# gabry1998/Self-Supervised-Anomaly-Detection

Hardware: AMD Instinct MI355X
Metric: train images/sec + anomaly-maps/sec, ResNet-18 256x256 bs256 (higher is better)
Workload: dtype f32; 1 GPU; ResNet-18 256x256 bs256 self-sup train + anomaly map, 1xMI355X, synthetic images (BASELINE configs[1]); images_per_gpu=256, global_batch=256, patches_per_image=841, bank_rows=588, parallelism=dp1 (256 images), train_step_launch=hipGraph segments, train_graph_segments=1

## Files before the change

### include/ssad.h

```cpp
#ifndef SSAD_H
#define SSAD_H
#include <stddef.h>
#include <stdint.h>

#ifdef __cplusplus
extern "C" {
#endif

#define SSAD_VERSION 100

int ssad_version(void);
const char* ssad_last_error(void);

int ssad_repack_oihw_to_ohwi(const float* w_oihw, float* w_ohwi, int O, int I, int KH, int KW, void* stream);
int ssad_repack_ohwi_to_oihw(const float* w_ohwi, float* w_oihw, int O, int I, int KH, int KW, void* stream);
int ssad_pack_stem_weight(const float* w_oihw, float* wk, void* stream);
int ssad_pack_stem_weight_ohwi(const float* w_ohwi, float* wk, void* stream);

int ssad_stem_fwd(const float* img, int B, int H, int W, int patch_dim, int patch_stride, int Hv, int Wv,
                  const float* wk, const float* scale, const float* shift, int relu, int hwnc, float* out, void* stream);
int ssad_stem_stats_rows(void);
int ssad_stem_fwd_stats(const float* img, int B, int H, int W, int Hv, int Wv, const float* wk, float* out, float eps,
                        float momentum, float* mean, float* invstd, float* running_mean, float* running_var, double* workspace,
                        void* stream);

int ssad_pack_stem_weight_folded(const float* w_oihw, float* wf, void* stream);
int ssad_stem_patch_pool_fwd(const float* img, int B, int H, int W, int patch_stride, const float* wf, const float* scale,
                             const float* shift, int hwnc, float* out, void* stream);
int ssad_stem_patch_pool_fwd_ring(const float* img, int B, int H, int W, int patch_stride, const float* wf, const float* scale,
                                  const float* shift, int hwnc, int skip_lo, int skip_hi, float* out, void* stream);
int ssad_stem_patch_border_fwd(const float* img, int B, int H, int W, int patch_stride, const float* wf, const float* scale,
                               const float* shift, float* out, void* stream);

int ssad_maxpool3x3s2_fwd(const float* in, float* out, int64_t N, int H, int W, int C, int hwnc, void* stream);

int ssad_conv_igemm_fwd(const float* in, const float* w_ohwi, float* out, const float* scale, const float* shift,
                        const float* residual, int relu, int64_t N, int H, int W, int Cin, int Cout, int KH, int KW,
                        int stride, int pad, void* stream);

int ssad_conv_igemm_fwd_hwnc(const float* in, const float* w_ohwi, float* out, const float* scale, const float* shift,
                             const float* residual, int relu, int64_t N, int H, int W, int Cin, int Cout, int KH, int KW,
                             int stride, int pad, void* stream);

int ssad_conv_igemm_fwd_hwnc_ring(const float* in, const float* w_ohwi, float* out, const float* scale, const float* shift,
                                  const float* residual, int relu, int64_t N, int H, int W, int Cin, int Cout, int KH, int KW,
                                  int stride, int pad, int skip_lo, int skip_hi, void* stream);
int ssad_patch_gather_hwnc(const float* dense, float* out, int64_t B, int prow, int pcol, int shift, int Hd, int Wd, int C,
                           int H, int W, int lo, int hi, void* stream);
int ssad_patch_gather_hwnc_band(const float* dense, float* out, int64_t B, int prow, int pcol, int shift, int Hd, int Wd, int C,
                                int H, int W, int lo, int hi, int ilo, int ihi, void* stream);

int ssad_conv_igemm_tile(int64_t N, int H, int W, int Cin, int Cout, int KH, int KW, int stride, int pad, int mode);
int ssad_conv_igemm_tile_id(int64_t N, int H, int W, int Cin, int Cout, int KH, int KW, int stride, int pad, int mode);

int ssad_gap_fwd(const float* in, float* out, int64_t N, int HW, int C, int out_stride, int out_offset, int hwnc,
// ... 376 lines not shown
```

### self-supervised-anomaly-detection_amd/csrc/stem.hip

```cpp
#include "common.h"
#include <type_traits>

namespace {

constexpr int STEM_MAX_GRID = 4096;


constexpr int TOH = 8, TOW = 32;
constexpr int TIH = TOH * 2 + 5;
constexpr int TIW = 72;
constexpr int KSTEPS = 7 * 4 * 3;
constexpr int IN_TILE = TIH * TIW * 3;
constexpr int W_TILE = KSTEPS * 2 * 64;

struct StemParams {
    const float* img;
    const float* wk;
    const float* scale;
    const float* shift;
    float* out;
    int B, H, W, pd, ps, Hv, Wv, Ho, Wo, relu;
    int prow, pcol;
    int ph, pw;
    int tiles_y, tiles_x;
// ... 168 lines not shown
            const int which = tid >> 6, cc = tid & 63;
            p.stats[((int64_t)blockIdx.x * 2 + which) * 64 + cc] =
                ((S[(0 * 2 + which) * 64 + cc] + S[(1 * 2 + which) * 64 + cc]) + S[(2 * 2 + which) * 64 + cc]) + S[(3 * 2 + which) * 64 + cc];
        }
    }
}

constexpr int SP_SW = 40, SP_SH = 36;
constexpr int SP_SRC = SP_SH * SP_SW * 3;
constexpr int SP_WF = 24 * 2 * 64;
constexpr int SP_CB = 9 * 32 * 32;

struct StemPatchParams {
    const float* img;
    const float* wf;
    const float* scale;
    const float* shift;
    float* out;
    int B, H, W, ps, prow, pcol, hwnc;
    int skip_lo, skip_hi;
    int64_t Nsamp;
};

__global__ __launch_bounds__(256, 2) void stem_patch_fused_kernel(StemPatchParams p) {
    extern __shared__ __attribute__((aligned(16))) float lds[];
    float* wl = lds;
    float* src = lds + SP_WF;
    float* cb = src + SP_SRC;
    const int tid = threadIdx.x, lane = tid & 63, wave = tid >> 6;
    const int r = lane & 31, h = lane >> 5;
    for (int i = tid; i < SP_WF / 4; i += 256) ((f32x4*)wl)[i] = ((const f32x4*)p.wf)[i];
    const int P = p.prow * p.pcol;
    const int64_t plane = (int64_t)p.H * p.W;

    constexpr int NSRC = (SP_SH * SP_SW + 255) / 256;
    float pv[NSRC][3];
    auto fetch_patch = [&](int64_t n) {
        const int b = (int)(n / P);
        const int pi = (int)(n - (int64_t)b * P);
        const int y0 = (pi / p.pcol) * p.ps, x0 = (pi % p.pcol) * p.ps;
        const float* im = p.img + (int64_t)b * 3 * plane;
#pragma unroll
        for (int q = 0; q < NSRC; ++q) {
            const int i = tid + 256 * q;
            const int ty = i / SP_SW, tx = i - ty * SP_SW;
            const int sy = ty - 2, sx = tx - 2;
            float v0 = 0.f, v1 = 0.f, v2 = 0.f;
            if (i < SP_SH * SP_SW && (unsigned)sy < 32u && (unsigned)sx < 32u) {
                const float* s = im + (int64_t)(y0 + sy) * p.W + x0 + sx;
                v0 = s[0]; v1 = s[plane]; v2 = s[2 * plane];
            }
            pv[q][0] = v0; pv[q][1] = v1; pv[q][2] = v2;
        }
    };
    if ((int64_t)blockIdx.x < p.Nsamp) fetch_patch(blockIdx.x);
    for (int64_t n = blockIdx.x; n < p.Nsamp; n += gridDim.x) {
        __syncthreads();
#pragma unroll
        for (int q = 0; q < NSRC; ++q) {
            const int i = tid + 256 * q;
            if (i < SP_SH * SP_SW) {
                float* d = src + i * 3;
                d[0] = pv[q][0]; d[1] = pv[q][1]; d[2] = pv[q][2];
            }
        }
        if (n + gridDim.x < p.Nsamp) fetch_patch(n + gridDim.x);
        for (int pass = 0; pass < 2; ++pass) {
            const float sc = p.scale ? p.scale[pass * 32 + r] : 1.f;
            const float sh = p.shift ? p.shift[pass * 32 + r] : 0.f;
            for (int i = tid; i < 32 * 32; i += 256) cb[i] = 0.f;
            __syncthreads();
            for (int t = 0; t < 4; ++t) {
                f32x16 acc0, acc1;
#pragma unroll
                for (int e = 0; e < 16; ++e) { acc0[e] = 0.f; acc1[e] = 0.f; }
                const int oy = 8 * t + 2 * wave;
                const float* a0 = src + ((oy + 0) * SP_SW + r + h) * 3;
                const float* a1 = src + ((oy + 1) * SP_SW + r + h) * 3;
                const float* bw = wl + h * 64 + pass * 32 + r;
#pragma unroll
                for (int a = 0; a < 4; ++a)
#pragma unroll
                    for (int q = 0; q < 2; ++q)
#pragma unroll
                        for (int c = 0; c < 3; ++c) {
                            const int ko = (a * SP_SW + 2 * q) * 3 + c;
                            const float w = bw[((a * 2 + q) * 3 + c) * 128];
                            acc0 = mfma32(a0[ko], w, acc0);
                            acc1 = mfma32(a1[ko], w, acc1);
                        }
                float* c0 = cb + ((1 + 2 * wave) * 32) * 32 + r;
#pragma unroll
                for (int e = 0; e < 16; ++e) {
                    const int ox = (e & 3) + 8 * (e >> 2) + 4 * h;
                    c0[ox * 32] = fmaxf(acc0[e] * sc + sh, 0.f);
                    c0[(32 + ox) * 32] = fmaxf(acc1[e] * sc + sh, 0.f);
                }
                __syncthreads();
#pragma unroll
                for (int k = 0; k < 2; ++k) {
                    const int item = tid + 256 * k;
                    const int c4 = item & 7, px = (item >> 3) & 15, j = item >> 7;
                    if (4 * t + j >= p.skip_lo && 4 * t + j <= p.skip_hi && px >= p.skip_lo && px <= p.skip_hi) continue;
                    f32x4 m = {0.f, 0.f, 0.f, 0.f};
#pragma unroll
                    for (int dy = 0; dy < 3; ++dy)
#pragma unroll
                        for (int dx = -1; dx < 2; ++dx) {
                            const int cx = 2 * px + dx;
                            if (cx < 0) continue;
                            const f32x4 v = *(const f32x4*)(cb + ((2 * j + dy) * 32 + cx) * 32 + c4 * 4);
                            m[0] = fmaxf(m[0], v[0]); m[1] = fmaxf(m[1], v[1]); m[2] = fmaxf(m[2], v[2]); m[3] = fmaxf(m[3], v[3]);
                        }
                    const int py = 4 * t + j;
                    const int64_t pix = p.hwnc ? ((int64_t)py * 16 + px) * p.Nsamp + n : (n * 16 + py) * 16 + px;
                    *(f32x4*)(p.out + pix * 64 + pass * 32 + c4 * 4) = m;
                }
                __syncthreads();
                ((f32x4*)cb)[tid] = ((const f32x4*)(cb + 8 * 32 * 32))[tid];
                __syncthreads();
            }
        }
    }
}

constexpr int SB_CB = 7 * 32 * 32;

__global__ __launch_bounds__(256, 2) void stem_patch_border_kernel(StemPatchParams p) {
    extern __shared__ __attribute__((aligned(16))) float lds[];
    float* wl = lds;
    float* src = lds + SP_WF;
    float* cb = src + SP_SRC;
    const int tid = threadIdx.x, lane = tid & 63, wave = tid >> 6;
    const int r = lane & 31, h = lane >> 5;
    for (int i = tid; i < SP_WF / 4; i += 256) ((f32x4*)wl)[i] = ((const f32x4*)p.wf)[i];
    const int P = p.prow * p.pcol;
    const int64_t plane = (int64_t)p.H * p.W;
    constexpr int NSRC = (SP_SH * SP_SW + 255) / 256;
    float pv[NSRC][3];
    auto fetch_patch = [&](int64_t n) {
        const int b = (int)(n / P);
        const int pi = (int)(n - (int64_t)b * P);
        const int y0 = (pi / p.pcol) * p.ps, x0 = (pi % p.pcol) * p.ps;
        const float* im = p.img + (int64_t)b * 3 * plane;
#pragma unroll
        for (int q = 0; q < NSRC; ++q) {
            const int i = tid + 256 * q;
            const int ty = i / SP_SW, tx = i - ty * SP_SW;
            const int sy = ty - 2, sx = tx - 2;
            float v0 = 0.f, v1 = 0.f, v2 = 0.f;
            if (i < SP_SH * SP_SW && (unsigned)sy < 32u && (unsigned)sx < 32u) {
                const float* s = im + (int64_t)(y0 + sy) * p.W + x0 + sx;
                v0 = s[0]; v1 = s[plane]; v2 = s[2 * plane];
            }
            pv[q][0] = v0; pv[q][1] = v1; pv[q][2] = v2;
        }
    };
    auto row_of = [](int t) { return t < 4 ? t : 25 + t; };
    const int ta0 = 2 * wave, ta1 = 2 * wave + 1 < 7 ? 2 * wave + 1 : 2 * wave;
    const float* pa0 = src + (row_of(ta0) * SP_SW + r + h) * 3;
    const float* pa1 = src + (row_of(ta1) * SP_SW + r + h) * 3;
    const float *pb0, *pb1;
    {
        int q0 = (2 * wave) * 32 + r, q1 = (2 * wave + 1) * 32 + r;
        q0 = q0 < 189 ? q0 : 188; q1 = q1 < 189 ? q1 : 188;
        const int c0 = q0 % 7, c1 = q1 % 7;
        pb0 = src + ((3 + q0 / 7) * SP_SW + (c0 < 4 ? c0 : 25 + c0) + h) * 3;
        pb1 = src + ((3 + q1 / 7) * SP_SW + (c1 < 4 ? c1 : 25 + c1) + h) * 3;
    }
    auto two_tiles = [&](const float* a0, const float* a1, int pass, f32x16& acc0, f32x16& acc1) {
#pragma unroll
        for (int e = 0; e < 16; ++e) { acc0[e] = 0.f; acc1[e] = 0.f; }
        const float* bw = wl + h * 64 + pass * 32 + r;
#pragma unroll
        for (int a = 0; a < 4; ++a)
#pragma unroll
            for (int q = 0; q < 2; ++q)
#pragma unroll
                for (int c = 0; c < 3; ++c) {
                    const int ko = (a * SP_SW + 2 * q) * 3 + c;
                    const float w = bw[((a * 2 + q) * 3 + c) * 128];
                    acc0 = mfma32(a0[ko], w, acc0);
                    acc1 = mfma32(a1[ko], w, acc1);
                }
    };
    if ((int64_t)blockIdx.x < p.Nsamp) fetch_patch(blockIdx.x);
    for (int64_t n = blockIdx.x; n < p.Nsamp; n += gridDim.x) {
        __syncthreads();
#pragma unroll
        for (int q = 0; q < NSRC; ++q) {
            const int i = tid + 256 * q;
            if (i < SP_SH * SP_SW) {
                float* d = src + i * 3;
                d[0] = pv[q][0]; d[1] = pv[q][1]; d[2] = pv[q][2];
            }
        }
        if (n + gridDim.x < p.Nsamp) fetch_patch(n + gridDim.x);
        __syncthreads();
        for (int pass = 0; pass < 2; ++pass) {
            const float sc = p.scale ? p.scale[pass * 32 + r] : 1.f;
            const float sh = p.shift ? p.shift[pass * 32 + r] : 0.f;
            f32x16 acc0, acc1;
            two_tiles(pa0, pa1, pass, acc0, acc1);
#pragma unroll
            for (int e = 0; e < 16; ++e) {
                const int ox = (e & 3) + 8 * (e >> 2) + 4 * h;
                cb[((2 * wave) * 32 + ox) * 32 + r] = fmaxf(acc0[e] * sc + sh, 0.f);
                if (2 * wave + 1 < 7) cb[((2 * wave + 1) * 32 + ox) * 32 + r] = fmaxf(acc1[e] * sc + sh, 0.f);
            }
            __syncthreads();
            for (int item = tid; item < 3 * 16 * 8; item += 256) {
                const int c4 = item & 7, px = (item >> 3) & 15, pr = item >> 7;
                const int t_lo = pr == 0 ? 0 : pr == 1 ? 1 : 4, t_hi = pr == 0 ? 1 : pr == 1 ? 3 : 6;
                f32x4 m = {0.f, 0.f, 0.f, 0.f};
                for (int t = t_lo; t <= t_hi; ++t)
#pragma unroll
                    for (int dx = -1; dx < 2; ++dx) {
                        const int cx = 2 * px + dx;
                        if (cx < 0) continue;
                        const f32x4 v = *(const f32x4*)(cb + (t * 32 + cx) * 32 + c4 * 4);
                        m[0] = fmaxf(m[0], v[0]); m[1] = fmaxf(m[1], v[1]); m[2] = fmaxf(m[2], v[2]); m[3] = fmaxf(m[3], v[3]);
                    }
                const int py = pr < 2 ? pr : 15;
                *(f32x4*)(p.out + (((int64_t)py * 16 + px) * p.Nsamp + n) * 64 + pass * 32 + c4 * 4) = m;
            }
            __syncthreads();
            if (wave < 3) {
                two_tiles(pb0, pb1, pass, acc0, acc1);
#pragma unroll
                for (int e = 0; e < 16; ++e) {
                    const int i = (e & 3) + 8 * (e >> 2) + 4 * h;
                    const int q0 = (2 * wave) * 32 + i, q1 = q0 + 32;
                    if (q0 < 189) cb[q0 * 32 + r] = fmaxf(acc0[e] * sc + sh, 0.f);
                    if (q1 < 189) cb[q1 * 32 + r] = fmaxf(acc1[e] * sc + sh, 0.f);
                }
            }
            __syncthreads();
            for (int item = tid; item < 13 * 3 * 8; item += 256) {
                const int c4 = item & 7, k = item >> 3, pk = k % 3, py = 2 + k / 3;
                const int ci_lo = pk == 0 ? 0 : pk == 1 ? 1 : 4, ci_hi = pk == 0 ? 1 : pk == 1 ? 3 : 6;
                f32x4 m = {0.f, 0.f, 0.f, 0.f};
#pragma unroll
                for (int dy = -1; dy < 2; ++dy)
                    for (int ci = ci_lo; ci <= ci_hi; ++ci) {
                        const f32x4 v = *(const f32x4*)(cb + ((2 * py + dy - 3) * 7 + ci) * 32 + c4 * 4);
                        m[0] = fmaxf(m[0], v[0]); m[1] = fmaxf(m[1], v[1]); m[2] = fmaxf(m[2], v[2]); m[3] = fmaxf(m[3], v[3]);
                    }
                const int px = pk < 2 ? pk : 15;
                *(f32x4*)(p.out + (((int64_t)py * 16 + px) * p.Nsamp + n) * 64 + pass * 32 + c4 * 4) = m;
            }
            __syncthreads();
        }
    }
}

__global__ void pack_stem_weight_folded_kernel(const float* __restrict__ w, float* __restrict__ wf) {
    const int i = blockIdx.x * blockDim.x + threadIdx.x;
    if (i >= SP_WF) return;
    const int co = i & 63, hh = (i >> 6) & 1, s = i >> 7;
    const int c = s % 3, q = (s / 3) & 1, a = s / 6;
    const int b = 2 * q + hh;
    const int ky0 = a == 0 ? 0 : 2 * a - 1, ky1 = a == 0 ? 0 : 2 * a;
    const int kx0 = b == 0 ? 0 : 2 * b - 1, kx1 = b == 0 ? 0 : 2 * b;
    float acc = 0.f;
    for (int ky = ky0; ky <= ky1; ++ky)
        for (int kx = kx0; kx <= kx1; ++kx) acc += w[((co * 3 + c) * 7 + ky) * 7 + kx];
    wf[i] = acc;
}

__global__ void pack_stem_weight_kernel(const float* __restrict__ w, float* __restrict__ wk, int ohwi = 0) {
    int i = blockIdx.x * blockDim.x + threadIdx.x;
    if (i >= 168 * 64) return;
    int co = i & 63, kl = i >> 6;
    int hh = kl & 1, rest = kl >> 1;
// ... 152 lines not shown
                                     running_var, stream);
}

extern "C" int ssad_pack_stem_weight_folded(const float* w_oihw, float* wf, void* stream) {
    SSAD_CHECK_ARG(w_oihw && wf, "null pointer");
    hipLaunchKernelGGL(pack_stem_weight_folded_kernel, dim3((SP_WF + 255) / 256), dim3(256), 0, (hipStream_t)stream, w_oihw, wf);
    SSAD_CHECK_LAUNCH();
    return 0;
}

extern "C" int ssad_stem_patch_pool_fwd_ring(const float* img, int B, int H, int W, int patch_stride, const float* wf,
                                             const float* scale, const float* shift, int hwnc, int skip_lo, int skip_hi, float* out,
                                             void* stream);
extern "C" int ssad_stem_patch_pool_fwd(const float* img, int B, int H, int W, int patch_stride, const float* wf,
                                        const float* scale, const float* shift, int hwnc, float* out, void* stream) {
    return ssad_stem_patch_pool_fwd_ring(img, B, H, W, patch_stride, wf, scale, shift, hwnc, 1, 0, out, stream);
}
extern "C" int ssad_stem_patch_pool_fwd_ring(const float* img, int B, int H, int W, int patch_stride, const float* wf,
                                             const float* scale, const float* shift, int hwnc, int skip_lo, int skip_hi, float* out,
                                             void* stream) {
    SSAD_CHECK_ARG(img && wf && out, "null pointer");
    SSAD_CHECK_ARG(skip_lo > skip_hi || (skip_lo >= 0 && skip_hi < 16), "skipped square outside the 16 x 16 map");
    SSAD_CHECK_ARG(B > 0 && H >= 32 && W >= 32 && patch_stride > 0, "bad shape (32x32 windows)");
    StemPatchParams p;
    p.img = img; p.wf = wf; p.scale = scale; p.shift = shift; p.out = out;
    p.B = B; p.H = H; p.W = W; p.ps = patch_stride; p.hwnc = hwnc; p.skip_lo = skip_lo; p.skip_hi = skip_hi;
    p.prow = (H - 32) / patch_stride + 1;
    p.pcol = (W - 32) / patch_stride + 1;
    p.Nsamp = (int64_t)B * p.prow * p.pcol;
    constexpr int lds_bytes = (SP_WF + SP_SRC + SP_CB) * 4;
    static bool attr_set = false;
    if (!attr_set) {
        SSAD_SET_DYN_LDS(stem_patch_fused_kernel, lds_bytes);
        attr_set = true;
    }
    const int64_t grid = p.Nsamp < 2048 ? p.Nsamp : 2048;
    hipLaunchKernelGGL(stem_patch_fused_kernel, dim3((unsigned)grid), dim3(256), lds_bytes, (hipStream_t)stream, p);
    SSAD_CHECK_LAUNCH();
    return 0;
}

extern "C" int ssad_stem_patch_border_fwd(const float* img, int B, int H, int W, int patch_stride, const float* wf, const float* scale,
                                          const float* shift, float* out, void* stream) {
    SSAD_CHECK_ARG(img && wf && out, "null pointer");
    SSAD_CHECK_ARG(B > 0 && H >= 32 && W >= 32 && patch_stride > 0, "bad shape (32x32 windows)");
    StemPatchParams p;
    p.img = img; p.wf = wf; p.scale = scale; p.shift = shift; p.out = out;
    p.B = B; p.H = H; p.W = W; p.ps = patch_stride; p.hwnc = 1; p.skip_lo = 1; p.skip_hi = 0;
    p.prow = (H - 32) / patch_stride + 1;
    p.pcol = (W - 32) / patch_stride + 1;
    p.Nsamp = (int64_t)B * p.prow * p.pcol;
    constexpr int lds_bytes = (SP_WF + SP_SRC + SB_CB) * 4;
    static bool attr_set = false;
    if (!attr_set) {
        SSAD_SET_DYN_LDS(stem_patch_border_kernel, lds_bytes);
        attr_set = true;
    }
    const int64_t grid = p.Nsamp < 2048 ? p.Nsamp : 2048;
    hipLaunchKernelGGL(stem_patch_border_kernel, dim3((unsigned)grid), dim3(256), lds_bytes, (hipStream_t)stream, p);
    SSAD_CHECK_LAUNCH();
    return 0;
}

template <typename T>
static int maxpool_fwd_impl(const T* in, T* out, uint8_t* idx, int64_t N, int H, int W, int C, int hwnc, void* stream,
                            PoolBN bn = PoolBN{nullptr, nullptr, nullptr, nullptr}, T* zwin = nullptr) {
    SSAD_CHECK_ARG(in && out, "null pointer");
    SSAD_CHECK_ARG(N > 0 && H > 0 && W > 0 && C > 0 && C % 4 == 0, "bad shape (C % 4)");
    int Ho = (H - 1) / 2 + 1, Wo = (W - 1) / 2 + 1;
    constexpr int E = Lane<T>::E;
    SSAD_CHECK_ARG(C % E == 0, "channel count must be a multiple of the 16-byte lane width");
    int64_t totalE = N * Ho * Wo * (C / E);
    SSAD_CHECK_ARG(cdiv64(totalE, 256) < (int64_t)2147483647, "too large");
    hipLaunchKernelGGL(maxpool3x3s2_kernel<T>, dim3((unsigned)cdiv64(totalE, 256)), dim3(256), 0, (hipStream_t)stream, in, out, idx,
                       totalE, H, W, C / E, Ho, Wo, N, hwnc, bn, zwin);
    SSAD_CHECK_LAUNCH();
    return 0;
}

extern "C" int ssad_bn_relu_maxpool_fwd(const float* z, const float* mean, const float* invstd, const float* gamma,
                                        const float* beta, float* out, uint8_t* idx, int64_t N, int H, int W, int C,
                                        void* stream) {
// ... 33 lines not shown
```

### self-supervised-anomaly-detection_amd/self_supervised/_hip.py

```python
import ctypes
import os

import torch

_HERE = os.path.dirname(os.path.abspath(__file__))
LIB_PATH = os.path.join(os.path.dirname(_HERE), "lib", "libssad_hip.so")

_c_fp = ctypes.c_void_p
_c_i = ctypes.c_int
_c_l = ctypes.c_int64
_c_f = ctypes.c_float

SIGNATURES = {
    "ssad_repack_oihw_to_ohwi": [_c_fp, _c_fp, _c_i, _c_i, _c_i, _c_i, _c_fp],
    "ssad_repack_ohwi_to_oihw": [_c_fp, _c_fp, _c_i, _c_i, _c_i, _c_i, _c_fp],
    "ssad_pack_stem_weight": [_c_fp, _c_fp, _c_fp],
    "ssad_pack_stem_weight_ohwi": [_c_fp, _c_fp, _c_fp],
    "ssad_pack_stem_weight16_ohwi": [_c_fp, _c_fp, _c_i, _c_fp],
    "ssad_stem_fwd": [_c_fp, _c_i, _c_i, _c_i, _c_i, _c_i, _c_i, _c_i, _c_fp, _c_fp, _c_fp, _c_i, _c_i, _c_fp, _c_fp],
    "ssad_stem_stats_rows": [],
    "ssad_stem_fwd_stats": [_c_fp, _c_i, _c_i, _c_i, _c_i, _c_i, _c_fp, _c_fp, _c_f, _c_f, _c_fp, _c_fp, _c_fp, _c_fp, _c_fp, _c_fp],
    "ssad_pack_stem_weight_folded": [_c_fp, _c_fp, _c_fp],
    "ssad_stem_patch_pool_fwd": [_c_fp, _c_i, _c_i, _c_i, _c_i, _c_fp, _c_fp, _c_fp, _c_i, _c_fp, _c_fp],
    "ssad_stem_patch_pool_fwd_ring": [_c_fp, _c_i, _c_i, _c_i, _c_i, _c_fp, _c_fp, _c_fp, _c_i, _c_i, _c_i, _c_fp, _c_fp],
    "ssad_stem_patch_border_fwd": [_c_fp, _c_i, _c_i, _c_i, _c_i, _c_fp, _c_fp, _c_fp, _c_fp, _c_fp],
    "ssad_maxpool3x3s2_fwd": [_c_fp, _c_fp, _c_l, _c_i, _c_i, _c_i, _c_i, _c_fp],
    "ssad_conv_igemm_fwd": [_c_fp, _c_fp, _c_fp, _c_fp, _c_fp, _c_fp, _c_i, _c_l, _c_i, _c_i, _c_i, _c_i, _c_i, _c_i,
                            _c_i, _c_i, _c_fp],
    "ssad_conv_igemm_fwd_hwnc": [_c_fp, _c_fp, _c_fp, _c_fp, _c_fp, _c_fp, _c_i, _c_l, _c_i, _c_i, _c_i, _c_i, _c_i, _c_i,
                                 _c_i, _c_i, _c_fp],
    "ssad_conv_igemm_fwd_hwnc_ring": [_c_fp, _c_fp, _c_fp, _c_fp, _c_fp, _c_fp, _c_i, _c_l, _c_i, _c_i, _c_i, _c_i, _c_i, _c_i,
                                      _c_i, _c_i, _c_i, _c_i, _c_fp],
    "ssad_patch_gather_hwnc": [_c_fp, _c_fp, _c_l, _c_i, _c_i, _c_i, _c_i, _c_i, _c_i, _c_i, _c_i, _c_i, _c_i, _c_fp],
    "ssad_patch_gather_hwnc_band": [_c_fp, _c_fp, _c_l, _c_i, _c_i, _c_i, _c_i, _c_i, _c_i, _c_i, _c_i, _c_i, _c_i, _c_i, _c_i, _c_fp],
    "ssad_conv_igemm_tile": [_c_l, _c_i, _c_i, _c_i, _c_i, _c_i, _c_i, _c_i, _c_i, _c_i],
    "ssad_conv_igemm_tile_id": [_c_l, _c_i, _c_i, _c_i, _c_i, _c_i, _c_i, _c_i, _c_i, _c_i],
    "ssad_gap_fwd": [_c_fp, _c_fp, _c_l, _c_i, _c_i, _c_i, _c_i, _c_i, _c_fp],
    "ssad_l2_normalize_rows": [_c_fp, _c_fp, _c_l, _c_i, _c_fp],
    "ssad_cosine_knn_mean": [_c_fp, _c_fp, _c_l, _c_i, _c_i, _c_fp],
    "ssad_cosine_knn_fused": [_c_fp, _c_fp, _c_fp, _c_l, _c_i, _c_i, _c_i, _c_fp],
    "ssad_cosine_knn_split": [_c_fp, _c_fp, _c_fp, _c_fp, _c_l, _c_i, _c_i, _c_i, _c_i, _c_fp],
    "ssad_cosine_knn_index": [_c_fp, _c_fp, _c_fp, _c_fp, _c_l, _c_i, _c_i, _c_i, _c_fp],
    "ssad_cosine_knn_index_split": [_c_fp, _c_fp, _c_fp, _c_fp, _c_fp, _c_l, _c_i, _c_i, _c_i, _c_i, _c_fp],
    "ssad_rows_smallest_index": [_c_fp, _c_l, _c_i, _c_i, _c_i, _c_i, _c_fp, _c_fp, _c_fp, _c_fp],
    "ssad_rows_argmax": [_c_fp, _c_l, _c_i, _c_fp, _c_fp, _c_fp],
    "ssad_knn_reweight": [_c_fp, _c_fp, _c_fp, _c_fp, _c_fp, _c_fp, _c_l, _c_i, _c_i, _c_i, _c_fp],
    "ssad_row_sqnorms": [_c_fp, _c_fp, _c_l, _c_i, _c_fp],
    "ssad_l2_knn_fused": [_c_fp, _c_fp, _c_fp, _c_fp, _c_l, _c_i, _c_i, _c_i, _c_fp],
# ... 250 lines not shown
```

### self-supervised-anomaly-detection_amd/self_supervised/engine.py

```python
import torch
from torch import nn

import os as _os

from . import ops

BLOCKS = [("layer1", 64, 64, 1), ("layer2", 64, 128, 2), ("layer3", 128, 256, 2), ("layer4", 256, 512, 2)]


def math_mode():
    m = _os.environ.get("SSAD_MATH", "f32").lower()
    return 6 if m in ("bf16x6", "x6") else 3 if m in ("bf16x3", "x3") else 0


class _Block(nn.Module):

    def __init__(self, cin, cout, stride):
        super().__init__()
        self.conv1 = nn.Conv2d(cin, cout, 3, stride, 1, bias=False)
        self.bn1 = nn.BatchNorm2d(cout)
        self.conv2 = nn.Conv2d(cout, cout, 3, 1, 1, bias=False)
        self.bn2 = nn.BatchNorm2d(cout)
        self.downsample = None
        if stride != 1 or cin != cout:
# ... 113 lines not shown
                    d["p1"], d["p2"] = ops.conv3x3_fw_pack_scaled(d["w1"], d["s1"]), ops.conv3x3_fw_pack_scaled(d["w2"], d["s2"])
                t = ops.conv3x3_fw_eval(a, d["p1"], 64, d["t1"], None, True, False)
                a = ops.conv3x3_fw_eval(t, d["p2"], 64, d["t2"], idt, True, hwnc and i == 1)
            else:
                t = ops.conv3x3_c64_eval(a, d["w1"], d["s1"], d["t1"], None, True, False, False)
                a = ops.conv3x3_c64_eval(t, d["w2"], d["s2"], d["t2"], idt, True, False, hwnc and i == 1, False)
        else:
            t = conv(a, d["w1"], d["s1"], d["t1"], None, True, s, 1)
        if not (c64 and name == "layer1"):
            a = conv(t, d["w2"], d["s2"], d["t2"], idt, True, 1, 1)
        last_of_stage = (i % 2 == 1)
        if last_of_stage and name in offs:
            ops.gap_fwd(a, pooled, offs[name], hwnc)
        if last_of_stage and maps is not None and name in maps:
            maps[name] = a
    return pooled


def _trunk_eval_dedup(plan, x, patch_stride, layer_outputs, pooled, conv):
    b, _, h, w = x.shape
    prow, pcol = (h - 32) // patch_stride + 1, (w - 32) // patch_stride + 1
    shift = patch_stride // 2
    band = _os.environ.get("SSAD_GATHER_BAND", "1") != "0"
    dn = ops.stem_fwd(x, plan.stem_w, plan.stem_s, plan.stem_t, True, resize_to=(2 * h, 2 * w))
    dn = ops.maxpool3x3s2_fwd(dn)
    if band and _os.environ.get("SSAD_STEM_BORDER", "1") != "0":
        a = ops.stem_patch_border_fwd(x, plan.stem_wf, plan.stem_s, plan.stem_t, patch_stride)
        ops.patch_gather_hwnc(dn, a, prow, pcol, shift, 2, 14, 4, 12)
    else:
        a = ops.stem_patch_pool_fwd(x, plan.stem_wf, plan.stem_s, plan.stem_t, patch_stride, True, (4, 12) if band else None)
    offs, off = {}, 0
    for k in ("layer1", "layer2", "layer3"):
        if k in layer_outputs:
            offs[k] = off
            off += {"layer1": 64, "layer2": 128, "layer3": 256}[k]
    offs["layer4"] = off
    for i, (name, d) in enumerate(plan.blocks):
        s = d["stride"]
        if name == "layer1":
            lo, hi = 3 + 2 * i, 13 - 2 * i
            dt = ops.conv3x3_c64_eval(dn, d["w1"], d["s1"], d["t1"], None, True)
            dn2 = ops.conv3x3_c64_eval(dt, d["w2"], d["s2"], d["t2"], dn, True)
            t = ops.conv_fwd_hwnc_ring(a, d["w1"], d["s1"], d["t1"], None, True, lo, hi)
            ops.patch_gather_hwnc(dt, t, prow, pcol, shift, lo, hi, *((lo + 2, hi - 2) if band else (1, 0)))
            a2 = ops.conv_fwd_hwnc_ring(t, d["w2"], d["s2"], d["t2"], a, True, lo + 1, hi - 1)
            ops.patch_gather_hwnc(dn2, a2, prow, pcol, shift, lo + 1, hi - 1, *((lo + 3, hi - 3) if band and i == 0 else (1, 0)))
            a, dn = a2, dn2
        else:
# ... 18 lines not shown
```

### self-supervised-anomaly-detection_amd/self_supervised/ops.py

```python
import os

import torch

from . import _hip


PROFILE = None


def _new(shape, like):
    return torch.empty(shape, device=like.device, dtype=torch.float32)


def _newh(shape, like):
    return torch.empty(shape, device=like.device, dtype=torch.float16)


def _is_h(t):
    return t is not None and t.dtype == torch.float16


def _p(t, allow_none=False):
    return _hip.ptr(t, allow_none, torch.float16 if _is_h(t) else torch.float32)

# ... 194 lines not shown
    out = _new((24, 2, 64), w)
    _hip.check(_hip.lib().ssad_pack_stem_weight_folded(_hip.ptr(w), _hip.ptr(out), _hip.stream()))
    return out


def stem_patch_pool_fwd(img, wf, scale, shift, patch_stride=8, hwnc=False, skip=None):
    b, c, h, w = img.shape
    n = b * ((h - 32) // patch_stride + 1) * ((w - 32) // patch_stride + 1)
    out = _new((16, 16, n, 64) if hwnc else (n, 16, 16, 64), img)
    lo, hi = skip if skip is not None else (1, 0)
    _run("stem_patch_pool", 2.0 * n * 32 * 32 * 64 * 147, 4.0 * (img.numel() + out.numel()),
         lambda: _hip.lib().ssad_stem_patch_pool_fwd_ring(_hip.ptr(img), b, h, w, patch_stride, _hip.ptr(wf), _hip.ptr(scale, True),
                                                          _hip.ptr(shift, True), int(hwnc), lo, hi, _hip.ptr(out), _hip.stream()))
    return out


def stem_patch_border_fwd(img, wf, scale, shift, patch_stride=8):
    b, c, h, w = img.shape
    n = b * ((h - 32) // patch_stride + 1) * ((w - 32) // patch_stride + 1)
    out = _new((16, 16, n, 64), img)
    _run("stem_patch_pool", 2.0 * n * 13 * 32 * 64 * 147, 4.0 * (img.numel() + out.numel() * 87 // 256),
         lambda: _hip.lib().ssad_stem_patch_border_fwd(_hip.ptr(img), b, h, w, patch_stride, _hip.ptr(wf), _hip.ptr(scale, True),
                                                       _hip.ptr(shift, True), _hip.ptr(out), _hip.stream()))
    return out


def maxpool3x3s2_fwd(x, hwnc=False):
    if hwnc:
        h, w, n, c = x.shape
        out = _new(((h - 1) // 2 + 1, (w - 1) // 2 + 1, n, c), x)
    else:
        n, h, w, c = x.shape
        out = _new((n, (h - 1) // 2 + 1, (w - 1) // 2 + 1, c), x)
    _run("maxpool3x3s2", 0.0, 4.0 * (x.numel() + out.numel()),
         lambda: _hip.lib().ssad_maxpool3x3s2_fwd(_hip.ptr(x), _hip.ptr(out), n, h, w, c, int(hwnc), _hip.stream()))
    return out


def _split_fwd(mode):
    return _hip.lib().ssad_conv_igemm_fwd_x6 if mode == 6 else _hip.lib().ssad_conv_igemm_fwd_x3


def conv_fwd_hwnc(x, w_ohwi, scale=None, shift=None, residual=None, relu=False, stride=1, pad=0, x3=False):
    h, w, n, cin = x.shape
    cout, kh, kw, cin2 = w_ohwi.shape
    assert cin == cin2
# ... 1745 lines not shown
```

Measured before the change: 8181 images/sec.

## Fuse dense stem conv with maxpool into a tiled kernel using buffer loads

```diff
diff --git a/include/ssad.h b/include/ssad.h
--- a/include/ssad.h
+++ b/include/ssad.h
@@ -31,6 +31,10 @@
                                   const float* shift, int hwnc, int skip_lo, int skip_hi, float* out, void* stream);
 int ssad_stem_patch_border_fwd(const float* img, int B, int H, int W, int patch_stride, const float* wf, const float* scale,
                                const float* shift, float* out, void* stream);
+
+int ssad_stem_dense_pool_ok(int H, int W);
+int ssad_stem_dense_pool_fwd(const float* img, int B, int H, int W, const float* wf, const float* scale, const float* shift,
+                             float* out, void* stream);
 
 int ssad_maxpool3x3s2_fwd(const float* in, float* out, int64_t N, int H, int W, int C, int hwnc, void* stream);
 
diff --git a/self-supervised-anomaly-detection_amd/csrc/stem.hip b/self-supervised-anomaly-detection_amd/csrc/stem.hip
--- a/self-supervised-anomaly-detection_amd/csrc/stem.hip
+++ b/self-supervised-anomaly-detection_amd/csrc/stem.hip
@@ -214,6 +214,67 @@
     int64_t Nsamp;
 };
 
+constexpr unsigned SP_OOB = 0x80000000u;
+constexpr int SP_SRD3 = 0x00020000;
+
+template <int ROWS>
+__device__ __forceinline__ void sp_fetch(float (&pv)[(ROWS * SP_SW + 255) / 256][3], const float* im, int plane, int W, int y0, int x0,
+                                         int ylo, int yhi, int xlo, int xhi, int tid) {
+    const __amdgpu_buffer_rsrc_t rs = __builtin_amdgcn_make_buffer_rsrc((void*)im, 0, (int)SP_OOB, SP_SRD3);
+#pragma unroll
+    for (int q = 0; q < (ROWS * SP_SW + 255) / 256; ++q) {
+        const int i = tid + 256 * q;
+        const int ty = i / SP_SW, tx = i - ty * SP_SW;
+        const int sy = y0 + ty, sx = x0 + tx;
+        const bool ok = i < ROWS * SP_SW && sy >= ylo && sy < yhi && sx >= xlo && sx < xhi;
+#pragma unroll
+        for (int c = 0; c < 3; ++c)
+            pv[q][c] = __builtin_bit_cast(float, __builtin_amdgcn_raw_buffer_load_b32(
+                rs, ok ? (unsigned)((sy * W + sx + c * plane) * 4) : SP_OOB, 0, 0));
+    }
+}
+
+template <int ROWS>
+__device__ __forceinline__ void sp_stage(float* src, const float (&pv)[(ROWS * SP_SW + 255) / 256][3], int tid) {
+#pragma unroll
+    for (int q = 0; q < (ROWS * SP_SW + 255) / 256; ++q) {
+        const int i = tid + 256 * q;
+        if (i < ROWS * SP_SW) {
+            float* d = src + i * 3;
+            d[0] = pv[q][0]; d[1] = pv[q][1]; d[2] = pv[q][2];
+        }
+    }
+}
+
+template <int NT>
+__device__ __forceinline__ void sp_tiles(const float* const (&a)[NT], const float* bw, f32x16 (&acc)[NT]) {
+#pragma unroll
+    for (int i = 0; i < NT; ++i)
+#pragma unroll
+        for (int e = 0; e < 16; ++e) acc[i][e] = 0.f;
+#pragma unroll
+    for (int ka = 0; ka < 4; ++ka)
+#pragma unroll
+        for (int q = 0; q < 2; ++q)
+#pragma unroll
+            for (int c = 0; c < 3; ++c) {
+                const int ko = (ka * SP_SW + 2 * q) * 3 + c;
+                const float w = bw[((ka * 2 + q) * 3 + c) * 128];
+#pragma unroll
+                for (int i = 0; i < NT; ++i) acc[i] = mfma32(a[i][ko], w, acc[i]);
+            }
+}
+
+__device__ __forceinline__ float sp_bn_relu(float v, float sc, float sh) { return fmaxf(v * sc + sh, 0.f); }
+
+__device__ __forceinline__ const float* sp_patch_origin(const StemPatchParams& p, int64_t n, int& y0, int& x0) {
+    const int P = p.prow * p.pcol;
+    const int b = (int)(n / P);
+    const int pi = (int)(n - (int64_t)b * P);
+    y0 = (pi / p.pcol) * p.ps; x0 = (pi % p.pcol) * p.ps;
+    return p.img + (int64_t)b * 3 * p.H * p.W;
+}
+
 __global__ __launch_bounds__(256, 2) void stem_patch_fused_kernel(StemPatchParams p) {
     extern __shared__ __attribute__((aligned(16))) float lds[];
     float* wl = lds;
@@ -222,40 +283,18 @@
     const int tid = threadIdx.x, lane = tid & 63, wave = tid >> 6;
     const int r = lane & 31, h = lane >> 5;
     for (int i = tid; i < SP_WF / 4; i += 256) ((f32x4*)wl)[i] = ((const f32x4*)p.wf)[i];
-    const int P = p.prow * p.pcol;
-    const int64_t plane = (int64_t)p.H * p.W;
 
     constexpr int NSRC = (SP_SH * SP_SW + 255) / 256;
     float pv[NSRC][3];
     auto fetch_patch = [&](int64_t n) {
-        const int b = (int)(n / P);
-        const int pi = (int)(n - (int64_t)b * P);
-        const int y0 = (pi / p.pcol) * p.ps, x0 = (pi % p.pcol) * p.ps;
-        const float* im = p.img + (int64_t)b * 3 * plane;
-#pragma unroll
-        for (int q = 0; q < NSRC; ++q) {
-            const int i = tid + 256 * q;
-            const int ty = i / SP_SW, tx = i - ty * SP_SW;
-            const int sy = ty - 2, sx = tx - 2;
-            float v0 = 0.f, v1 = 0.f, v2 = 0.f;
-            if (i < SP_SH * SP_SW && (unsigned)sy < 32u && (unsigned)sx < 32u) {
-                const float* s = im + (int64_t)(y0 + sy) * p.W + x0 + sx;
-                v0 = s[0]; v1 = s[plane]; v2 = s[2 * plane];
-            }
-            pv[q][0] = v0; pv[q][1] = v1; pv[q][2] = v2;
-        }
+        int y0, x0;
+        const float* im = sp_patch_origin(p, n, y0, x0);
+        sp_fetch<SP_SH>(pv, im, p.H * p.W, p.W, y0 - 2, x0 - 2, y0, y0 + 32, x0, x0 + 32, tid);
     };
     if ((int64_t)blockIdx.x < p.Nsamp) fetch_patch(blockIdx.x);
     for (int64_t n = blockIdx.x; n < p.Nsamp; n += gridDim.x) {
         __syncthreads();
-#pragma unroll
-        for (int q = 0; q < NSRC; ++q) {
-            const int i = tid + 256 * q;
-            if (i < SP_SH * SP_SW) {
-                float* d = src + i * 3;
-                d[0] = pv[q][0]; d[1] = pv[q][1]; d[2] = pv[q][2];
-            }
-        }
+        sp_stage<SP_SH>(src, pv, tid);
         if (n + gridDim.x < p.Nsamp) fetch_patch(n + gridDim.x);
         for (int pass = 0; pass < 2; ++pass) {
             const float sc = p.scale ? p.scale[pass * 32 + r] : 1.f;
@@ -263,30 +302,16 @@
             for (int i = tid; i < 32 * 32; i += 256) cb[i] = 0.f;
             __syncthreads();
             for (int t = 0; t < 4; ++t) {
-                f32x16 acc0, acc1;
-#pragma unroll
-                for (int e = 0; e < 16; ++e) { acc0[e] = 0.f; acc1[e] = 0.f; }
+                f32x16 acc[2];
                 const int oy = 8 * t + 2 * wave;
-                const float* a0 = src + ((oy + 0) * SP_SW + r + h) * 3;
-                const float* a1 = src + ((oy + 1) * SP_SW + r + h) * 3;
-                const float* bw = wl + h * 64 + pass * 32 + r;
-#pragma unroll
-                for (int a = 0; a < 4; ++a)
-#pragma unroll
-                    for (int q = 0; q < 2; ++q)
-#pragma unroll
-                        for (int c = 0; c < 3; ++c) {
-                            const int ko = (a * SP_SW + 2 * q) * 3 + c;
-                            const float w = bw[((a * 2 + q) * 3 + c) * 128];
-                            acc0 = mfma32(a0[ko], w, acc0);
-                            acc1 = mfma32(a1[ko], w, acc1);
-                        }
+                const float* const a[2] = {src + ((oy + 0) * SP_SW + r + h) * 3, src + ((oy + 1) * SP_SW + r + h) * 3};
+                sp_tiles<2>(a, wl + h * 64 + pass * 32 + r, acc);
                 float* c0 = cb + ((1 + 2 * wave) * 32) * 32 + r;
 #pragma unroll
                 for (int e = 0; e < 16; ++e) {
                     const int ox = (e & 3) + 8 * (e >> 2) + 4 * h;
-                    c0[ox * 32] = fmaxf(acc0[e] * sc + sh, 0.f);
-                    c0[(32 + ox) * 32] = fmaxf(acc1[e] * sc + sh, 0.f);
+                    c0[ox * 32] = sp_bn_relu(acc[0][e], sc, sh);
+                    c0[(32 + ox) * 32] = sp_bn_relu(acc[1][e], sc, sh);
                 }
                 __syncthreads();
 #pragma unroll
@@ -326,27 +351,12 @@
     const int tid = threadIdx.x, lane = tid & 63, wave = tid >> 6;
     const int r = lane & 31, h = lane >> 5;
     for (int i = tid; i < SP_WF / 4; i += 256) ((f32x4*)wl)[i] = ((const f32x4*)p.wf)[i];
-    const int P = p.prow * p.pcol;
-    const int64_t plane = (int64_t)p.H * p.W;
     constexpr int NSRC = (SP_SH * SP_SW + 255) / 256;
     float pv[NSRC][3];
     auto fetch_patch = [&](int64_t n) {
-        const int b = (int)(n / P);
-        const int pi = (int)(n - (int64_t)b * P);
-        const int y0 = (pi / p.pcol) * p.ps, x0 = (pi % p.pcol) * p.ps;
-        const float* im = p.img + (int64_t)b * 3 * plane;
-#pragma unroll
-        for (int q = 0; q < NSRC; ++q) {
-            const int i = tid + 256 * q;
-            const int ty = i / SP_SW, tx = i - ty * SP_SW;
-            const int sy = ty - 2, sx = tx - 2;
-            float v0 = 0.f, v1 = 0.f, v2 = 0.f;
-            if (i < SP_SH * SP_SW && (unsigned)sy < 32u && (unsigned)sx < 32u) {
-                const float* s = im + (int64_t)(y0 + sy) * p.W + x0 + sx;
-                v0 = s[0]; v1 = s[plane]; v2 = s[2 * plane];
-            }
-            pv[q][0] = v0; pv[q][1] = v1; pv[q][2] = v2;
-        }
+        int y0, x0;
+        const float* im = sp_patch_origin(p, n, y0, x0);
+        sp_fetch<SP_SH>(pv, im, p.H * p.W, p.W, y0 - 2, x0 - 2, y0, y0 + 32, x0, x0 + 32, tid);
     };
     auto row_of = [](int t) { return t < 4 ? t : 25 + t; };
     const int ta0 = 2 * wave, ta1 = 2 * wave + 1 < 7 ? 2 * wave + 1 : 2 * wave;
@@ -360,45 +370,25 @@
         pb0 = src + ((3 + q0 / 7) * SP_SW + (c0 < 4 ? c0 : 25 + c0) + h) * 3;
         pb1 = src + ((3 + q1 / 7) * SP_SW + (c1 < 4 ? c1 : 25 + c1) + h) * 3;
     }
-    auto two_tiles = [&](const float* a0, const float* a1, int pass, f32x16& acc0, f32x16& acc1) {
-#pragma unroll
-        for (int e = 0; e < 16; ++e) { acc0[e] = 0.f; acc1[e] = 0.f; }
-        const float* bw = wl + h * 64 + pass * 32 + r;
-#pragma unroll
-        for (int a = 0; a < 4; ++a)
-#pragma unroll
-            for (int q = 0; q < 2; ++q)
-#pragma unroll
-                for (int c = 0; c < 3; ++c) {
-                    const int ko = (a * SP_SW + 2 * q) * 3 + c;
-                    const float w = bw[((a * 2 + q) * 3 + c) * 128];
-                    acc0 = mfma32(a0[ko], w, acc0);
-                    acc1 = mfma32(a1[ko], w, acc1);
-                }
-    };
+    const float* const pa[2] = {pa0, pa1};
+    const float* const pb[2] = {pb0, pb1};
     if ((int64_t)blockIdx.x < p.Nsamp) fetch_patch(blockIdx.x);
     for (int64_t n = blockIdx.x; n < p.Nsamp; n += gridDim.x) {
         __syncthreads();
-#pragma unroll
-        for (int q = 0; q < NSRC; ++q) {
-            const int i = tid + 256 * q;
-            if (i < SP_SH * SP_SW) {
-                float* d = src + i * 3;
-                d[0] = pv[q][0]; d[1] = pv[q][1]; d[2] = pv[q][2];
-            }
-        }
+        sp_stage<SP_SH>(src, pv, tid);
         if (n + gridDim.x < p.Nsamp) fetch_patch(n + gridDim.x);
         __syncthreads();
         for (int pass = 0; pass < 2; ++pass) {
             const float sc = p.scale ? p.scale[pass * 32 + r] : 1.f;
             const float sh = p.shift ? p.shift[pass * 32 + r] : 0.f;
-            f32x16 acc0, acc1;
-            two_tiles(pa0, pa1, pass, acc0, acc1);
+            const float* bw = wl + h * 64 + pass * 32 + r;
+            f32x16 acc[2];
+            sp_tiles<2>(pa, bw, acc);
 #pragma unroll
             for (int e = 0; e < 16; ++e) {
                 const int ox = (e & 3) + 8 * (e >> 2) + 4 * h;
-                cb[((2 * wave) * 32 + ox) * 32 + r] = fmaxf(acc0[e] * sc + sh, 0.f);
-                if (2 * wave + 1 < 7) cb[((2 * wave + 1) * 32 + ox) * 32 + r] = fmaxf(acc1[e] * sc + sh, 0.f);
+                cb[((2 * wave) * 32 + ox) * 32 + r] = sp_bn_relu(acc[0][e], sc, sh);
+                if (2 * wave + 1 < 7) cb[((2 * wave + 1) * 32 + ox) * 32 + r] = sp_bn_relu(acc[1][e], sc, sh);
             }
             __syncthreads();
             for (int item = tid; item < 3 * 16 * 8; item += 256) {
@@ -418,13 +408,13 @@
             }
             __syncthreads();
             if (wave < 3) {
-                two_tiles(pb0, pb1, pass, acc0, acc1);
+                sp_tiles<2>(pb, bw, acc);
 #pragma unroll
                 for (int e = 0; e < 16; ++e) {
                     const int i = (e & 3) + 8 * (e >> 2) + 4 * h;
                     const int q0 = (2 * wave) * 32 + i, q1 = q0 + 32;
-                    if (q0 < 189) cb[q0 * 32 + r] = fmaxf(acc0[e] * sc + sh, 0.f);
-                    if (q1 < 189) cb[q1 * 32 + r] = fmaxf(acc1[e] * sc + sh, 0.f);
+                    if (q0 < 189) cb[q0 * 32 + r] = sp_bn_relu(acc[0][e], sc, sh);
+                    if (q1 < 189) cb[q1 * 32 + r] = sp_bn_relu(acc[1][e], sc, sh);
                 }
             }
             __syncthreads();
@@ -442,6 +432,103 @@
                 *(f32x4*)(p.out + (((int64_t)py * 16 + px) * p.Nsamp + n) * 64 + pass * 32 + c4 * 4) = m;
             }
             __syncthreads();
+        }
+    }
+}
+
+struct StemDenseParams {
+    const float* img;
+    const float* wf;
+    const float* scale;
+    const float* shift;
+    float* out;
+    int B, H, W, Hp, Wp;
+    int uy, ux;
+    int64_t units;
+};
+
+__global__ __launch_bounds__(256, 2) void stem_dense_pool_kernel(StemDenseParams p) {
+    extern __shared__ __attribute__((aligned(16))) float lds[];
+    float* wl = lds;
+    float* src = lds + SP_WF;
+    float* cb = src + SP_SRC;
+    const int tid = threadIdx.x, lane = tid & 63, wave = tid >> 6;
+    const int r = lane & 31, h = lane >> 5;
+    for (int i = tid; i < SP_WF / 4; i += 256) ((f32x4*)wl)[i] = ((const f32x4*)p.wf)[i];
+    const int per_image = p.uy * p.ux;
+
+    constexpr int NSRC = (SP_SH * SP_SW + 255) / 256;
+    float pv[NSRC][3];
+    auto fetch_unit = [&](int64_t u) {
+        const int b = (int)(u / per_image);
+        const int ui = (int)(u - (int64_t)b * per_image);
+        const int ty = ui / p.ux, tx = ui - ty * p.ux;
+        sp_fetch<SP_SH>(pv, p.img + (int64_t)b * 3 * p.H * p.W, p.H * p.W, p.W, 32 * ty - 3, 30 * tx - 3, 0, p.H, 0, p.W, tid);
+    };
+    if ((int64_t)blockIdx.x < p.units) fetch_unit(blockIdx.x);
+    for (int64_t u = blockIdx.x; u < p.units; u += gridDim.x) {
+        const int b = (int)(u / per_image);
+        const int ui = (int)(u - (int64_t)b * per_image);
+        const int ty = ui / p.ux, tx = ui - ty * p.ux;
+        __syncthreads();
+        sp_stage<SP_SH>(src, pv, tid);
+        if (u + gridDim.x < p.units) fetch_unit(u + gridDim.x);
+        const int nsteps = p.Hp - 16 * ty >= 16 ? 4 : (p.Hp - 16 * ty + 3) / 4;
+        const int cmin = tx == 0 ? 1 : 0;
+        float* const ob = p.out + (int64_t)b * p.Hp * p.Wp * 64;
+        for (int pass = 0; pass < 2; ++pass) {
+            const float sc = p.scale ? p.scale[pass * 32 + r] : 1.f;
+            const float sh = p.shift ? p.shift[pass * 32 + r] : 0.f;
+            const float* bw = wl + h * 64 + pass * 32 + r;
+            __syncthreads();
+            for (int t = 0; t < nsteps; ++t) {
+                const int k = 8 * t + 1 + 2 * wave;
+                float* c0 = cb + ((1 + 2 * wave) * 32) * 32 + r;
+                if (t == 0 && wave == 0 && ty > 0) {
+                    f32x16 acc[3];
+                    const float* const a[3] = {src + ((k + 0) * SP_SW + r + h) * 3, src + ((k + 1) * SP_SW + r + h) * 3, src + (r + h) * 3};
+                    sp_tiles<3>(a, bw, acc);
+#pragma unroll
+                    for (int e = 0; e < 16; ++e) {
+                        const int ox = (e & 3) + 8 * (e >> 2) + 4 * h;
+                        c0[ox * 32] = sp_bn_relu(acc[0][e], sc, sh);
+                        c0[(32 + ox) * 32] = sp_bn_relu(acc[1][e], sc, sh);
+                        cb[ox * 32 + r] = sp_bn_relu(acc[2][e], sc, sh);
+                    }
+                } else {
+                    f32x16 acc[2];
+                    const float* const a[2] = {src + ((k + 0) * SP_SW + r + h) * 3, src + ((k + 1) * SP_SW + r + h) * 3};
+                    sp_tiles<2>(a, bw, acc);
+#pragma unroll
+                    for (int e = 0; e < 16; ++e) {
+                        const int ox = (e & 3) + 8 * (e >> 2) + 4 * h;
+                        c0[ox * 32] = sp_bn_relu(acc[0][e], sc, sh);
+                        c0[(32 + ox) * 32] = sp_bn_relu(acc[1][e], sc, sh);
+                    }
+                }
+                __syncthreads();
+                const int smin = ty == 0 && t == 0 ? 1 : 0;
+#pragma unroll
+                for (int kk = 0; kk < 2; ++kk) {
+                    const int item = tid + 256 * kk;
+                    const int c4 = item & 7, kx = (item >> 3) & 15, j = item >> 7;
+                    const int py = 16 * ty + 4 * t + j, px = 15 * tx + kx;
+                    if (kx == 15 || py >= p.Hp || px >= p.Wp) continue;
+                    f32x4 m = {0.f, 0.f, 0.f, 0.f};
+#pragma unroll
+                    for (int dy = 0; dy < 3; ++dy)
+#pragma unroll
+                        for (int dx = 0; dx < 3; ++dx) {
+                            const int s = 2 * j + dy < smin ? smin : 2 * j + dy, cx = 2 * kx + dx < cmin ? cmin : 2 * kx + dx;
+                            const f32x4 v = *(const f32x4*)(cb + (s * 32 + cx) * 32 + c4 * 4);
+                            m[0] = fmaxf(m[0], v[0]); m[1] = fmaxf(m[1], v[1]); m[2] = fmaxf(m[2], v[2]); m[3] = fmaxf(m[3], v[3]);
+                        }
+                    *(f32x4*)(ob + ((int64_t)py * p.Wp + px) * 64 + pass * 32 + c4 * 4) = m;
+                }
+                __syncthreads();
+                ((f32x4*)cb)[tid] = ((const f32x4*)(cb + 8 * 32 * 32))[tid];
+                __syncthreads();
+            }
         }
     }
 }
@@ -640,6 +727,7 @@
     SSAD_CHECK_ARG(img && wf && out, "null pointer");
     SSAD_CHECK_ARG(skip_lo > skip_hi || (skip_lo >= 0 && skip_hi < 16), "skipped square outside the 16 x 16 map");
     SSAD_CHECK_ARG(B > 0 && H >= 32 && W >= 32 && patch_stride > 0, "bad shape (32x32 windows)");
+    SSAD_CHECK_ARG((int64_t)H * W * 12 < (int64_t)SP_OOB, "image beyond 32-bit byte offsets");
     StemPatchParams p;
     p.img = img; p.wf = wf; p.scale = scale; p.shift = shift; p.out = out;
     p.B = B; p.H = H; p.W = W; p.ps = patch_stride; p.hwnc = hwnc; p.skip_lo = skip_lo; p.skip_hi = skip_hi;
@@ -662,6 +750,7 @@
                                           const float* shift, float* out, void* stream) {
     SSAD_CHECK_ARG(img && wf && out, "null pointer");
     SSAD_CHECK_ARG(B > 0 && H >= 32 && W >= 32 && patch_stride > 0, "bad shape (32x32 windows)");
+    SSAD_CHECK_ARG((int64_t)H * W * 12 < (int64_t)SP_OOB, "image beyond 32-bit byte offsets");
     StemPatchParams p;
     p.img = img; p.wf = wf; p.scale = scale; p.shift = shift; p.out = out;
     p.B = B; p.H = H; p.W = W; p.ps = patch_stride; p.hwnc = 1; p.skip_lo = 1; p.skip_hi = 0;
@@ -676,6 +765,32 @@
     }
     const int64_t grid = p.Nsamp < 2048 ? p.Nsamp : 2048;
     hipLaunchKernelGGL(stem_patch_border_kernel, dim3((unsigned)grid), dim3(256), lds_bytes, (hipStream_t)stream, p);
+    SSAD_CHECK_LAUNCH();
+    return 0;
+}
+
+extern "C" int ssad_stem_dense_pool_ok(int H, int W) {
+    return H >= 32 && W >= 32 && H % 4 == 0 && W % 4 == 0 && (int64_t)H * W * 12 < (int64_t)SP_OOB;
+}
+
+extern "C" int ssad_stem_dense_pool_fwd(const float* img, int B, int H, int W, const float* wf, const float* scale, const float* shift,
+                                        float* out, void* stream) {
+    SSAD_CHECK_ARG(img && wf && out, "null pointer");
+    SSAD_CHECK_ARG(B > 0 && ssad_stem_dense_pool_ok(H, W), "bad shape (ssad_stem_dense_pool_ok)");
+    StemDenseParams p;
+    p.img = img; p.wf = wf; p.scale = scale; p.shift = shift; p.out = out;
+    p.B = B; p.H = H; p.W = W; p.Hp = H / 2; p.Wp = W / 2;
+    p.uy = (p.Hp + 15) / 16;
+    p.ux = (p.Wp + 14) / 15;
+    p.units = (int64_t)B * p.uy * p.ux;
+    constexpr int lds_bytes = (SP_WF + SP_SRC + SP_CB) * 4;
+    static bool attr_set = false;
+    if (!attr_set) {
+        SSAD_SET_DYN_LDS(stem_dense_pool_kernel, lds_bytes);
+        attr_set = true;
+    }
+    const int64_t grid = p.units < 2048 ? p.units : 2048;
+    hipLaunchKernelGGL(stem_dense_pool_kernel, dim3((unsigned)grid), dim3(256), lds_bytes, (hipStream_t)stream, p);
     SSAD_CHECK_LAUNCH();
     return 0;
 }
diff --git a/self-supervised-anomaly-detection_amd/self_supervised/_hip.py b/self-supervised-anomaly-detection_amd/self_supervised/_hip.py
--- a/self-supervised-anomaly-detection_amd/self_supervised/_hip.py
+++ b/self-supervised-anomaly-detection_amd/self_supervised/_hip.py
@@ -24,6 +24,8 @@
     "ssad_stem_patch_pool_fwd": [_c_fp, _c_i, _c_i, _c_i, _c_i, _c_fp, _c_fp, _c_fp, _c_i, _c_fp, _c_fp],
     "ssad_stem_patch_pool_fwd_ring": [_c_fp, _c_i, _c_i, _c_i, _c_i, _c_fp, _c_fp, _c_fp, _c_i, _c_i, _c_i, _c_fp, _c_fp],
     "ssad_stem_patch_border_fwd": [_c_fp, _c_i, _c_i, _c_i, _c_i, _c_fp, _c_fp, _c_fp, _c_fp, _c_fp],
+    "ssad_stem_dense_pool_ok": [_c_i, _c_i],
+    "ssad_stem_dense_pool_fwd": [_c_fp, _c_i, _c_i, _c_i, _c_fp, _c_fp, _c_fp, _c_fp, _c_fp],
     "ssad_maxpool3x3s2_fwd": [_c_fp, _c_fp, _c_l, _c_i, _c_i, _c_i, _c_i, _c_fp],
     "ssad_conv_igemm_fwd": [_c_fp, _c_fp, _c_fp, _c_fp, _c_fp, _c_fp, _c_i, _c_l, _c_i, _c_i, _c_i, _c_i, _c_i, _c_i,
                             _c_i, _c_i, _c_fp],
diff --git a/self-supervised-anomaly-detection_amd/self_supervised/engine.py b/self-supervised-anomaly-detection_amd/self_supervised/engine.py
--- a/self-supervised-anomaly-detection_amd/self_supervised/engine.py
+++ b/self-supervised-anomaly-detection_amd/self_supervised/engine.py
@@ -159,8 +159,11 @@
     prow, pcol = (h - 32) // patch_stride + 1, (w - 32) // patch_stride + 1
     shift = patch_stride // 2
     band = _os.environ.get("SSAD_GATHER_BAND", "1") != "0"
-    dn = ops.stem_fwd(x, plan.stem_w, plan.stem_s, plan.stem_t, True, resize_to=(2 * h, 2 * w))
-    dn = ops.maxpool3x3s2_fwd(dn)
+    if _os.environ.get("SSAD_STEM_DENSE", "1") != "0" and ops.stem_dense_pool_ok(h, w):
+        dn = ops.stem_dense_pool_fwd(x, plan.stem_wf, plan.stem_s, plan.stem_t)
+    else:
+        dn = ops.stem_fwd(x, plan.stem_w, plan.stem_s, plan.stem_t, True, resize_to=(2 * h, 2 * w))
+        dn = ops.maxpool3x3s2_fwd(dn)
     if band and _os.environ.get("SSAD_STEM_BORDER", "1") != "0":
         a = ops.stem_patch_border_fwd(x, plan.stem_wf, plan.stem_s, plan.stem_t, patch_stride)
         ops.patch_gather_hwnc(dn, a, prow, pcol, shift, 2, 14, 4, 12)
diff --git a/self-supervised-anomaly-detection_amd/self_supervised/ops.py b/self-supervised-anomaly-detection_amd/self_supervised/ops.py
--- a/self-supervised-anomaly-detection_amd/self_supervised/ops.py
+++ b/self-supervised-anomaly-detection_amd/self_supervised/ops.py
@@ -240,6 +240,21 @@
     _run("stem_patch_pool", 2.0 * n * 13 * 32 * 64 * 147, 4.0 * (img.numel() + out.numel() * 87 // 256),
          lambda: _hip.lib().ssad_stem_patch_border_fwd(_hip.ptr(img), b, h, w, patch_stride, _hip.ptr(wf), _hip.ptr(scale, True),
                                                        _hip.ptr(shift, True), _hip.ptr(out), _hip.stream()))
+    return out
+
+
+def stem_dense_pool_ok(h, w):
+    return bool(_hip.lib().ssad_stem_dense_pool_ok(int(h), int(w)))
+
+
+def stem_dense_pool_fwd(img, wf, scale, shift):
+    b, c, h, w = img.shape
+    assert c == 3
+    out = _new((b, h // 2, w // 2, 64), img)
+    _run("stem_dense_pool", 2.0 * b * h * w * 64 * 147, 4.0 * (img.numel() + out.numel()),
+         lambda: _hip.lib().ssad_stem_dense_pool_fwd(_hip.ptr(img), b, h, w, _hip.ptr(wf), _hip.ptr(scale, True), _hip.ptr(shift, True),
+                                                     _hip.ptr(out), _hip.stream()),
+         exec_flops=2.0 * b * h * w * 64 * 48)
     return out
 
 
```

Result: no change. 8164 images/sec (-0.2%).
